# AndrewCullacino/handwritten-chinese-ocr-samples

Hardware: AMD Instinct MI355X
Metric: text-lines/sec (1x128x2000 synth) greedy decode (higher is better)
Workload: dtype f16 (f32 accumulate); 1 GPU; BASELINE configs[1]: 64 x 1x128x2000 uint8 lines, random-init hctr checkpoint (C=7358), forward + greedy CTC decode, labels to host; global_lines=64, lines_per_gpu=64, width=2000, classes=7358, checkpoint=random, parallelism=batch-shard x1

## Files before the change

### handwritten-chinese-ocr-samples_amd/_lib.py

```python
import ctypes
import os
import subprocess
import sys

PKG_DIR = os.path.dirname(os.path.abspath(__file__))
ROOT = os.path.dirname(PKG_DIR)
CSRC = os.path.join(PKG_DIR, "csrc")
LIB_PATH = os.path.join(PKG_DIR, "libhctr_hip.so")
HEADER = os.path.join(ROOT, "include", "hctr_hip.h")

SOURCES = [("gather.cpp", ["-x", "hip"]), ("kernels.hip", []), ("preprocess.hip", ["-ffp-contract=off"]), ("engine.cpp", ["-x", "hip"]), ("beam_search.cpp", ["-ffp-contract=off"]),
           ("ngram_lm.cpp", ["-ffp-contract=off"])]
COMMON = ["--offload-arch=gfx950", "-O3", "-std=c++17", "-fPIC", "-Wall", "-Wno-unused-function"]

HCTR_OK = 0
ERR_ARG, ERR_HIP, ERR_STATE, ERR_KEY, ERR_SHAPE, ERR_EMPTY_LINE, ERR_NOMEM = -1, -2, -3, -4, -5, -6, -7
U8, F32, I64 = 0, 1, 2


def _deps():
    return [os.path.join(CSRC, s) for s, _ in SOURCES] + [os.path.join(CSRC, "kernels.h"),
                                                          os.path.join(CSRC, "ngram_lm.h"), HEADER]


# ... 92 lines not shown
LM_NEXT_CB = ctypes.CFUNCTYPE(ctypes.c_int, ctypes.c_void_p, ctypes.c_int, c_i32p, c_i32p, ctypes.c_int, c_i32p)


class BeamParams(ctypes.Structure):
    _fields_ = [("skip_search", ctypes.c_int), ("beam_size", ctypes.c_int), ("search_depth", ctypes.c_int),
                ("lm_panelty", ctypes.c_double), ("len_bonus", ctypes.c_double),
                ("builtin_lm", ctypes.c_int), ("label_codepoints", ctypes.c_void_p),
                ("score_cb", LM_SCORE_CB), ("next_cb", LM_NEXT_CB), ("user", ctypes.c_void_p),
                ("num_threads", ctypes.c_int), ("ngram", ctypes.c_void_p), ("label_words", ctypes.c_void_p)]


_VP, _I, _I64 = ctypes.c_void_p, ctypes.c_int, ctypes.c_int64
SIGNATURES = [
    ("hctr_create", _I, [ctypes.POINTER(_VP), _I, _I]),
    ("hctr_destroy", None, [_VP]),
    ("hctr_last_error", ctypes.c_char_p, [_VP]),
    ("hctr_version", ctypes.c_char_p, []),
    ("hctr_load_tensor", _I, [_VP, ctypes.c_char_p, _VP, c_i64p, _I, _I]),
    ("hctr_finalize_weights", _I, [_VP]),
    ("hctr_set_precision", _I, [_VP, _I]),
    ("hctr_set_guard", _I, [_VP, ctypes.c_double, ctypes.c_double]),
    ("hctr_last_guard", _I, [_VP, c_i64p, c_i64p, _VP, _VP, _VP, _I64]),
    ("hctr_lines_per_pass", _I, [_VP, _I, _I, _I]),
    ("hctr_workspace_stats", _I, [_VP, c_i64p, c_i64p, c_i64p]),
    ("hctr_forward_logits", _I, [_VP, _VP, _I, _I, _VP, _I, _I, _VP, _I]),
    ("hctr_greedy", _I, [_VP, _VP, _I, _I, _VP, _I, _I, _VP, _VP]),
    ("hctr_decode_greedy_logits", _I, [_VP, _VP, _I, _I, _I, _I, _VP, _VP]),
    ("hctr_beam_frontend", _I, [_VP, _VP, _I, _I, _VP, _VP, _I, _I, _I, _I, _I, _I, _VP, _VP, _VP, c_i64p]),
    ("hctr_beam_fetch_candidates", _I, [_VP, _VP, _VP, _VP]),
    ("hctr_log_softmax", _I, [_VP, _VP, _I, _I, _I, _I, _VP]),
    ("hctr_ctc_loss", _I, [_VP, _VP, _I, _I, _VP, _I, _I, _VP, _VP, _VP, _VP]),
    ("hctr_ctc_loss_logits", _I, [_VP, _VP, _I, _I, _I, _I, _VP, _VP, _VP, _VP]),
    ("hctr_ctc_loss_logits_grad", _I, [_VP, _VP, _I, _I, _I, _I, _VP, _VP, _VP, _VP, _VP, _VP, _I]),
    ("hctr_ctc_align", _I, [_VP, _VP, _I, _I, _VP, _I, _I, _VP, _VP, _VP, _VP, _VP, _VP, _VP, _VP]),
    ("hctr_ctc_align_logits", _I, [_VP, _VP, _I, _I, _I, _I, _VP, _VP, _VP, _VP, _VP, _VP, _VP, _VP]),
    ("hctr_recognize", _I, [_VP, _VP, _I, _I, _VP, _I, _I, _VP, _VP, _VP, _VP, _VP, _VP, _VP, _VP, _VP]),
    ("hctr_recognize_logits", _I, [_VP, _VP, _I, _I, _I, _I, _VP, _VP, _VP, _VP, _VP, _VP, _VP, _VP, _VP]),
    ("hctr_beam_search", _I, [ctypes.POINTER(BeamParams), _I, _I, _I, _I, _VP, _VP, _VP, _VP, _VP, _VP, _VP,
                              _VP, _VP, _VP]),
    ("hctr_ngram_load", _I, [ctypes.c_char_p, ctypes.POINTER(_VP)]),
    ("hctr_ngram_free", None, [_VP]),
    ("hctr_ngram_order", _I, [_VP]),
    ("hctr_ngram_word_id", ctypes.c_int32, [_VP, ctypes.c_char_p]),
    ("hctr_ngram_score", ctypes.c_double, [_VP, ctypes.c_char_p, _I, _I]),
    ("hctr_ngram_last_error", ctypes.c_char_p, []),
    ("hctr_comm_unique_id", _I, [_VP]),
# ... 83 lines not shown
```

### handwritten-chinese-ocr-samples_amd/csrc/engine.cpp

```cpp
#include "../../include/hctr_hip.h"
#include "kernels.h"

#include <algorithm>
#include <cfloat>
#include <cmath>
#include <cstdarg>
#include <cstdio>
#include <cstring>
#include <map>
#include <new>
#include <string>
#include <vector>

using namespace hctr;

namespace {

constexpr int kImgH = 128;
constexpr int kFeat = 2048;
constexpr double kBnEps = 1e-5;
constexpr int kStagePlanes[4] = {128, 256, 512, 512};
constexpr int kStageBlocks[4] = {2, 4, 5, 1};
constexpr int kStageH[5] = {128, 64, 32, 16, 8};
constexpr int64_t kDefaultMaxCols = 131072;
// ... 107 lines not shown
    bool big_tiles = true;
    int halo_mode = 2;
    int mode = 0;
    bool split = false;
    int x3_mask = 31;
    int out_class = 8;
    double guard_rel = 0.01, guard_abs = 0.05;
    std::vector<float> g_margin, g_scale;
    std::vector<uint8_t> g_flag;
    int64_t g_flagged_total = 0, g_lines_total = 0;
    std::vector<std::vector<int32_t>> h_widths;
    std::vector<int32_t> h_labels, h_lengths;
    char* pin = nullptr;
    size_t pin_cap = 0;
    int chm() const { return split ? 3 : 1; }
    bool fuse_se = true;
    std::string stamp_layer;
    unsigned long long* stamp_buf = nullptr;
    int64_t stamp_cap = 0, stamp_n = 0;
    bool fuse_ds = true;
    bool fuse_argmax = true;
    bool persist_dynamic = false;
    int conv_seq = 0;
    bool fuse_stem = true;
    bool fuse_beam = true;
    int64_t beam_fallbacks = 0;
    bool profiling = false;
    std::vector<ProfEntry> prof;
    std::vector<hipEvent_t> ev_pool;
    size_t ev_used = 0;
    std::vector<void*> beam_allocs;
    std::vector<int64_t> cand_off;
    std::vector<int32_t> cand_idx;
    std::vector<float> cand_logp;
    char* ctc_buf = nullptr;
    size_t ctc_cap = 0;
};

namespace {

int fail(hctr_ctx* c, int code, const char* fmt, ...) {
    char buf[1024];
    va_list ap;
    va_start(ap, fmt);
    vsnprintf(buf, sizeof(buf), fmt, ap);
    va_end(ap);
// ... 452 lines not shown
        a.ds_in_sh = ws.Wa * ds->cin;
        a.ds_in_sb = (int64_t)(in.H + 2) * ws.Wa * ds->cin;
    }
    a.mtiles = ws.B * a.tilesH * a.tilesW;
    a.ntiles = cw.coutPad / conv_tile_couts(tile);
    if (c->persist_dynamic && c->conv_seq < 64) a.tile_counter = ws.tile_ctrs + 8 * c->conv_seq++;
    if (c->stamp_buf && c->stamp_layer == name && (tile == TILE_HALO4 || tile == TILE_HALO4_8x32) &&
        (int64_t)a.mtiles * a.ntiles <= c->stamp_cap) {
        a.stamps = c->stamp_buf;
        c->stamp_n = (int64_t)a.mtiles * a.ntiles;
    }
    static const char* dbg_layer = getenv("HCTR_DBG_LAYER");
    if (dbg_layer && strcmp(dbg_layer, name) == 0)
        if (const char* e = getenv("HCTR_DBG")) a.dbg = atoi(e);
    pf.begin(name);
    if (stem_img_f32 >= 0) {
        if (tile != TILE_64x256 || cw.taps != 9 || cw.cin != 64 || cw.coutPad != 64 || c->split)
            return fail(c, HCTR_ERR_STATE, "conv %s: stem fusion not applicable", name);
        a.img = ws.img; a.img_f32 = stem_img_f32; a.img_widths = stem_widths ? ws.widths : nullptr;
        a.stem_w = c->wts().stem_w; a.stem_b = c->wts().stem_b;
        HIP_TRY(c, launch_stem_conv0_2(a, c->stream));
    } else {
        HIP_TRY(c, launch_conv(a, tile, cw.taps, false, c->stream));
    }
    pf.end();
    return HCTR_OK;
}

int run_block(hctr_ctx* c, Prof& pf, const std::string& name, const BlockW& bw, ActDesc in, half_t* t,
              half_t* o, half_t* r, int planes) {
    const Workspace& ws = c->ws;
    const int H = in.H;
    auto tiles_of = [&](const ConvW& cw) {
        const ConvTile t = pick_tile(c, cw, H);
        return (H / conv_tile_rows(t)) * ((ws.W + conv_tile_cols(t) - 1) / conv_tile_cols(t));
    };
    const float inv_hw = 1.0f / ((float)H * (float)ws.W);
    const half_t* res = in.p;
    const bool fuse_ds = bw.has_ds && c->fuse_ds && (c->fuse_se || c->split) && bw.ds.cin % kBK == 0 &&
                         pick_tile(c, bw.conv2, H) == TILE_HALO4;
    if (bw.has_ds && !fuse_ds) {
        c->out_class = 4;
        TRY(run_conv(c, pf, (name + ".downsample").c_str(), bw.ds, in, r, H, false, false, nullptr, false));
        res = r;
    }
    if (c->fuse_se || c->split) {
// ... 720 lines not shown

int hctr_last_guard(hctr_ctx* c, int64_t* lines, int64_t* flagged, uint8_t* flags, float* min_margin, float* scale,
                    int64_t cap) {
    return guard(c, [&]() -> int {
        if (!c) return HCTR_ERR_ARG;
        const int64_t n = (int64_t)c->g_flag.size();
        int64_t nf = 0;
        for (uint8_t f : c->g_flag) nf += f ? 1 : 0;
        if (lines) *lines = n;
        if (flagged) *flagged = nf;
        const int64_t m = n < cap ? n : (cap < 0 ? 0 : cap);
        if (flags && m) memcpy(flags, c->g_flag.data(), (size_t)m);
        if (min_margin && m) memcpy(min_margin, c->g_margin.data(), (size_t)m * 4);
        if (scale && m) memcpy(scale, c->g_scale.data(), (size_t)m * 4);
        return HCTR_OK;
    });
}

int hctr_workspace_stats(hctr_ctx* c, int64_t* arena_bytes, int64_t* arena_allocations, int64_t* recarves) {
    if (!c) return HCTR_ERR_ARG;
    if (arena_bytes) *arena_bytes = (int64_t)c->arena_cap;
    if (arena_allocations) *arena_allocations = c->arena_reallocs;
    if (recarves) *recarves = c->ws_recarves;
    return HCTR_OK;
}

int hctr_lines_per_pass(hctr_ctx* c, int B, int W, int f16x3) {
    return guard(c, [&]() -> int {
        if (!c) return HCTR_ERR_ARG;
        if (B < 1 || W < 1) return fail(c, HCTR_ERR_ARG, "bad batch shape B=%d W=%d", B, W);
        return sub_batch(c, B, W, f16x3 != 0);
    });
}

int hctr_set_profiling(hctr_ctx* c, int enabled) {
    if (!c) return HCTR_ERR_ARG;
    c->profiling = enabled != 0;
    return HCTR_OK;
}

int hctr_last_profile(hctr_ctx* c, char* names_buf, int cap, float* ms, int max_n) {
    return guard(c, [&]() -> int {
        if (!c) return HCTR_ERR_ARG;
        HIP_TRY(c, hipStreamSynchronize(c->stream));
        std::string names;
        std::vector<std::string> order;
// ... 809 lines not shown
```

### handwritten-chinese-ocr-samples_amd/csrc/kernels.h

```cpp
#pragma once
#include <hip/hip_runtime.h>
#include <stdint.h>

namespace hctr {

typedef _Float16 half_t;

constexpr int kTileW = 16;
constexpr int kBK = 64;

struct ConvArgs {
    const half_t* x;
    const half_t* w;
    const float* bias;
    void* y;
    float* se_part;
    const float* se_scale;
    const half_t* resid;
    int H, W;
    int Cin, Cout, CoutPad;
    int tilesW, tilesH;
    int64_t in_sb;
    int in_sh;
    int64_t out_sb;
// ... 23 lines not shown
    const float* stem_w;
    const float* stem_b;
    int split;
    int drop_lo;
    const half_t* ds_x;
    const half_t* ds_w;
    const float* ds_bias;
    int ds_cin;
    int ds_in_sh;
    int64_t ds_in_sb;
    int32_t* tile_counter;
    unsigned long long* stamps;
    int dbg;
};

enum ConvTile { TILE_64x256 = 0, TILE_128x128 = 1, TILE_256x256 = 2, TILE_HALO4 = 3, TILE_HALO4_8x32 = 4 };
inline int conv_tile_rows(ConvTile t) { return (t == TILE_128x128 || t == TILE_HALO4_8x32) ? 8 : 16; }
inline int conv_tile_cols(ConvTile t) { return t == TILE_HALO4_8x32 ? 32 : 16; }
inline int conv_tile_couts(ConvTile t) {
    return t == TILE_64x256 ? 64 : (t == TILE_256x256 ? 256 : 128);
}

hipError_t launch_conv(const ConvArgs& a, ConvTile tile, int taps, bool linear_f32, hipStream_t s);
constexpr int kLinearWN = 2;
hipError_t launch_argmax_partials(const float* val, const int32_t* cls, int P, int64_t M, int32_t* idx, hipStream_t s,
                                  const float* val2 = nullptr, const float* absp = nullptr, float* margin = nullptr,
                                  float* rowabs = nullptr);
hipError_t launch_row_guard(const float* logits, int64_t ld, int64_t M, int C, float* margin, float* rowabs, hipStream_t s);
hipError_t launch_line_guard(const float* margin, const float* rowabs, int B, int W, float* out, hipStream_t s);
size_t conv_lds_bytes(ConvTile tile);

hipError_t launch_stem_conv0_2(const ConvArgs& a, hipStream_t s);

hipError_t launch_zero_borders(half_t* p, int B, int H, int W, int Wa, int C, hipStream_t s);

hipError_t launch_stem(const void* img, int img_f32, const int32_t* widths_dev, const float* w9,
                       const float* bias, half_t* y, int B, int W, int Wa, int split, hipStream_t s);

hipError_t launch_se_border(const half_t* t, int B, int H, int W, int Wa, int C, int split, const float* tsum_part,
                            int tiles, float* out, hipStream_t s);
hipError_t launch_se_premean(const float* border, const half_t* t, const half_t* w, const float* bias, int B, int H,
                             int W, int Wa, int C, int CoutPad, int split, float* mean, const float* w1,
                             const float* w2, float* scale, int32_t* counter, hipStream_t s);

hipError_t launch_se_fc(const float* se_part, int tiles_per_img, const float* w1, const float* w2,
                        float* scale, int B, int C, float inv_hw, hipStream_t s);
// ... 86 lines not shown
```

### handwritten-chinese-ocr-samples_amd/csrc/kernels.hip

```cpp
#include "kernels.h"

#include <algorithm>
#include <cstdlib>

namespace hctr {

typedef _Float16 f16x8 __attribute__((ext_vector_type(8)));
typedef float f32x4 __attribute__((ext_vector_type(4)));
typedef float f32x2 __attribute__((ext_vector_type(2)));
typedef _Float16 f16x2 __attribute__((ext_vector_type(2)));
typedef uint32_t u32x4 __attribute__((ext_vector_type(4)));
typedef void __attribute__((address_space(3))) * lptr_t;

__device__ __forceinline__ void glds16_asm(const char* gsrc, char* lds_dst) {
    const uint32_t lds = (uint32_t)(uintptr_t)((lptr_t)lds_dst);
    uint32_t keep;
    asm volatile("s_mov_b32 %0, m0\n\ts_mov_b32 m0, %2\n\ts_nop 0\n\tglobal_load_lds_dwordx4 %1, off\n\ts_mov_b32 m0, %0"
                 : "=&s"(keep)
                 : "v"(gsrc), "s"(lds)
                 : "memory");
}

template <int CTRL>
__device__ __forceinline__ float dpp_f32(float v) {
// ... 27 lines not shown
                 : "v"(voff), "s"(s0), "s"(s1), "s"(s2), "s"(s3), "s"(l0), "s"(l1), "s"(l2), "s"(l3)
                 : "memory");
}

template <int LSTRIDE>
__device__ __forceinline__ void glds16x4v_asm_s(const char* sbase, uint32_t v0, uint32_t v1, uint32_t v2, uint32_t v3, char* d0) {
    const uint32_t l0 = (uint32_t)(uintptr_t)((lptr_t)d0);
    uint32_t keep;
    asm volatile("s_mov_b32 %0, m0\n\t"
                 "s_mov_b32 m0, %6\n\ts_nop 0\n\tglobal_load_lds_dwordx4 %1, %5\n\t"
                 "s_add_u32 m0, m0, %7\n\ts_nop 0\n\tglobal_load_lds_dwordx4 %2, %5\n\t"
                 "s_add_u32 m0, m0, %7\n\ts_nop 0\n\tglobal_load_lds_dwordx4 %3, %5\n\t"
                 "s_add_u32 m0, m0, %7\n\ts_nop 0\n\tglobal_load_lds_dwordx4 %4, %5\n\t"
                 "s_mov_b32 m0, %0"
                 : "=&s"(keep)
                 : "v"(v0), "v"(v1), "v"(v2), "v"(v3), "s"(sbase), "s"(l0), "i"(LSTRIDE)
                 : "memory", "scc");
}

__device__ __forceinline__ constexpr int acc_cout_offset(int j) { return (j >> 2) * 64 + ((j >> 1) & 1) * 32 + (j & 1) * 4; }

constexpr float kSeScaleFloor = 1e-12f;

template <int WN, int WM, int JT, bool LINEAR, bool SPLIT, bool PRIVATE_RED = false, bool BIAS_DONE = false,
          bool RESID_IN_ACC = false>
__device__ __forceinline__ void conv_epilogue(const ConvArgs& a, f32x4 (&acc)[JT][4], char* smem, int tid, int lane,
                                              int wn, int wm, int n0, int mt, int img, int th, int tw, int hbase,
                                              int w0, unsigned long long* st = nullptr) {
    auto estamp = [&](int i) {
        if (st != nullptr) {
            __builtin_amdgcn_sched_barrier(0);
            if (tid == 0) st[i] = __builtin_amdgcn_s_memrealtime();
            __builtin_amdgcn_sched_barrier(0);
        }
    };
    constexpr int WC = JT * 16;
    constexpr int BN = WN * WC, BM = WM * 64;
    const int q = lane >> 4;
    const int c = lane & 15;
    const int cw0 = n0 + wn * WC + q * 8;
    auto co = [](int j) { return acc_cout_offset(j); };

    if (!BIAS_DONE) {
#pragma unroll
        for (int j = 0; j < JT; ++j) {
            const f32x4 b4 = *(const f32x4*)(a.bias + cw0 + co(j));
#pragma unroll
            for (int n = 0; n < 4; ++n)
#pragma unroll
                for (int i = 0; i < 4; ++i) acc[j][n][i] += b4[i];
        }
// ... 130 lines not shown
            for (int cb = 0; cb < JT / 4; ++cb)
#pragma unroll
                for (int n = 0; n < 4; ++n) {
                    const half_t* r = a.resid + pix0 + (int64_t)(hbase + n) * a.out_sh + cb * 64;
                    const f16x8 h0 = *(const f16x8*)r, h1 = *(const f16x8*)(r + 32);
                    const f16x8 l0 = *(const f16x8*)(r + a.Cout), l1 = *(const f16x8*)(r + a.Cout + 32);
#pragma unroll
                    for (int e = 0; e < 16; ++e) {
                        const float rv = e < 8 ? (float)h0[e] + (float)l0[e] : (float)h1[e - 8] + (float)l1[e - 8];
                        const float sv = sc[cb * 64 + (e >> 3) * 32 + (e & 7)];
                        acc[cb * 4 + (e >> 2)][n][e & 3] = fmaf(acc[cb * 4 + (e >> 2)][n][e & 3], sv, rv);
                    }
                }
        }
    } else if (RESID_IN_ACC) {
        const float* sc = a.se_scale + (int64_t)img * a.Cout + cw0;
#pragma unroll
        for (int j = 0; j < JT; ++j) {
            const f32x4 s4 = *(const f32x4*)(sc + co(j));
#pragma unroll
            for (int n = 0; n < 4; ++n)
#pragma unroll
                for (int i = 0; i < 4; ++i) acc[j][n][i] *= fmaxf(s4[i], kSeScaleFloor);
        }
    } else if (a.se_scale != nullptr) {
        const float* sc = a.se_scale + (int64_t)img * a.Cout + cw0;
        if (w < a.out_wlimit) {
            f16x8 rlo[JT / 4][4], rhi[JT / 4][4];
#pragma unroll
            for (int cb = 0; cb < JT / 4; ++cb)
#pragma unroll
                for (int n = 0; n < 4; ++n) {
                    const half_t* r = a.resid + pix0 + (int64_t)(hbase + n) * a.out_sh + cb * 64;
                    rlo[cb][n] = *(const f16x8*)r;
                    rhi[cb][n] = *(const f16x8*)(r + 32);
                }
#pragma unroll
            for (int j = 0; j < JT; ++j) {
                const f32x4 s4 = *(const f32x4*)(sc + co(j));
#pragma unroll
                for (int n = 0; n < 4; ++n)
#pragma unroll
                    for (int i = 0; i < 4; ++i) {
                        const int e = (j & 3) * 4 + i;
                        const float r = e < 8 ? (float)rlo[j >> 2][n][e] : (float)rhi[j >> 2][n][e - 8];
                        acc[j][n][i] = fmaf(acc[j][n][i], s4[i], r);
// ... 562 lines not shown
                __builtin_amdgcn_s_setprio(0);
                __builtin_amdgcn_sched_barrier(0);
            }
        }
    }
    asm volatile("s_waitcnt vmcnt(0)" ::: "memory");
    conv_epilogue<WN, WM, JT, false, false>(a, acc, smem, tid, lane, wn, wm, n0, mt, img, th, tw, th * 16 + wm * 4,
                                            tw * 16);
}

namespace halo4_lds {
constexpr int kWeightBuf = 16384;
constexpr int kWeights = 0;
constexpr int kHalo = kWeights + 2 * kWeightBuf;
constexpr int kScratch = kHalo + kHaloBytes;
constexpr int kScratchBytes = 4 * 128 * 4;
constexpr int kHaloTable = kScratch;
constexpr int kHaloTableBytes = 4 * 12 * 8 * 4;
constexpr int kNextTile = kScratch + kScratchBytes;
constexpr int kTotal = kNextTile + 16;
static_assert(kHaloTableBytes <= kScratchBytes, "the halo-offset table fits inside the epilogue scratch it aliases");
static_assert(kNextTile >= kScratch + kScratchBytes, "the next-tile words lie behind the epilogue scratch");
static_assert(kTotal <= 80 * 1024, "two workgroups per CU on 160 KB of LDS");
}

template <int GEOM, bool SPLIT, bool PERSIST, bool STAMP = false, bool DSFUSE = false, bool RESPRE = false>
__global__ __launch_bounds__(256, 2) void conv3x3_halo4_kernel(const ConvArgs a) {
    static_assert(!DSFUSE || !PERSIST, "downsample fusion: non-persistent instances only");
    static_assert(!RESPRE || (!DSFUSE && !PERSIST && !SPLIT), "residual-in-prologue: plain f16 instances only");
    constexpr int WN = 1, WM = 4, JT = 8, BN = 128;
    constexpr int TR = GEOM ? 8 : 16, TC = GEOM ? 32 : 16;
    constexpr int S = TC + 4;
    static_assert((TR + 2) * S * 128 == kHaloBytes, "halo footprint");
    extern __shared__ __attribute__((aligned(16))) char smem[];
    const int tid = threadIdx.x;
    auto stamp = [&](int i) {
        if (STAMP && tid == 0) a.stamps[(size_t)blockIdx.x * 16 + i] = __builtin_amdgcn_s_memrealtime();
    };
    stamp(0);
    const int lane = tid & 63;
    const int wv = __builtin_amdgcn_readfirstlane(tid >> 6);
    const int wm = wv;
    const int cin = a.Cin;
    const int nkc = (a.dbg & 64) ? 0 : cin / kBK;
    const int nk = 9 * nkc;
    constexpr bool kPrefetch = !PERSIST && !STAMP && !RESPRE;
    static_assert(!(kPrefetch && PERSIST), "the halo-offset table aliases the epilogue scratch: one tile per workgroup");
    constexpr int kRing = 3;
    constexpr int kBhalfAt = 1;
    constexpr int kBpreAt = 4;
    constexpr int kEarlyAt = 1;

// ... 84 lines not shown
#pragma unroll
            for (int r = 0; r < 12; ++r) htab[(wv * 12 + r) * 8 + (lane >> 3)] = hoff[r] - cp0;
        }
    };
    const int hbuf = halo4_lds::kHalo + wrow * (S * 128);
    int bx[3][2];
#pragma unroll
    for (int d = 0; d < 3; ++d) {
        const int u = wcol + c + d;
        const int v0 = u * 128 + (((q ^ (u & 7)) & 7) << 4);
        bx[d][0] = hbuf + v0;
        bx[d][1] = hbuf + (v0 ^ 64);
    }
    auto b_ptrs = [&](int tap, const char*& be, const char*& bo) {
        const int tdy = tap / 3, d = tap - tdy * 3;
        be = smem + bx[d][tdy & 1] + tdy * (S * 128);
        bo = smem + bx[d][(tdy & 1) ^ 1] + tdy * (S * 128);
    };

    Tile cur = tile_at(tidx);
    int kbase = 0;
    bool first = true;

    int tile_no = 0;
    for (;;) {
        const bool has_next = PERSIST && (tnext < xcnt);
        const char* nxb = cur.xb;
        const char* nwb = cur.wb;
        if (has_next) {
            const Tile t = tile_at(tnext);
            nxb = t.xb;
            nwb = t.wb;
        }
        int drawn = 0;
        if (dynamic && tid == 0)
            drawn = 2 * nloc + __hip_atomic_fetch_add(a.tile_counter + xcd, 1, __ATOMIC_RELAXED, __HIP_MEMORY_SCOPE_AGENT);
        f32x4 acc[JT][4];
        f16x8 bq[2][4];
        auto mma_step = [&](const char* wt, const char* be, const char* bo, auto&& stage_next, auto&& after_group,
                            bool have_b0 = false, const char* nbe = nullptr, const char* nbo = nullptr,
                            int bhalf_at = kBhalfAt) {
            f16x8 ar[kRing][2];
            auto read_a = [&](int g, f16x8 (&dst)[2]) {
                const int ks = g >> 2, jp = g & 3;
                const char* base = wt + (ks ? aoff1 : aoff0);
                dst[0] = *(const f16x8*)(base + (2 * jp) * 2048);
// ... 143 lines not shown

        __builtin_amdgcn_s_waitcnt(0xc07f);
        __builtin_amdgcn_s_setprio(1);
        for (int kc = 0; kc < nkc; ++kc) {
            const bool next_chunk = kc + 1 < nkc;
#pragma unroll
            for (int tap = 0; tap < 9; ++tap) {
                const int k = kc * 9 + tap;
                asm volatile("s_waitcnt vmcnt(0)" ::: "memory");
                if (!(a.dbg & 1024)) __builtin_amdgcn_s_barrier();
                asm volatile("" ::: "memory");
                const char *be, *bo;
                b_ptrs(tap, be, bo);
                const bool more = k + 1 < nk;
                const bool wrap = tap == 8;
                const int tap1 = more ? (wrap ? 0 : tap + 1) : 0;
                const int kc1 = more ? (wrap ? kc + 1 : kc) : 0;
                const char* wsrc = more ? cur.wb : nwb;
                const char *nbe = nullptr, *nbo = nullptr;
                if (kPrefetch && tap < 8) b_ptrs(tap + 1, nbe, nbo);
                mma_step(weight_buf(kbase + k), be, bo, [&] {
                    if ((more || has_next) && !(a.dbg & 512))
                        stage_weights(wsrc, kc1, tap1, (kbase + k + 1) & 1);
                }, [&](int g) {
                    if (kPrefetch && tap == 8 && g == kEarlyAt && next_chunk) {
                        asm volatile("s_waitcnt lgkmcnt(0)" ::: "memory");
                        __builtin_amdgcn_s_barrier();
                        asm volatile("" ::: "memory");
                        static_assert(kHaloPieces == 45, "halo piece count");
                        const char* hsrc = (next_chunk ? cur.xb + (int64_t)(kc + 1) * (kBK * 2) : nxb);
                        char* d = smem + halo4_lds::kHalo + wv * 1024;
                        int ln = lane;
                        asm volatile("" : "+v"(ln));
                        const uint32_t* hrow = (const uint32_t*)(smem + halo4_lds::kHaloTable) + wv * 96 + (ln >> 3);
                        const uint32_t cpl = (uint32_t)((ln ^ (ln >> 3)) & 7) << 4;
                        uint32_t ho[4];
#pragma unroll
                        for (int r = 0; r < 4; ++r) ho[r] = hrow[r * 8] + cpl;
                        glds16x4v_asm_s<4096>(hsrc, ho[0], ho[1], ho[2], ho[3], d);
#pragma unroll
                        for (int r = 0; r < 4; ++r) ho[r] = hrow[(4 + r) * 8] + cpl;
                        glds16x4v_asm_s<4096>(hsrc, ho[0], ho[1], ho[2], ho[3], d + 4 * 4096);
#pragma unroll
                        for (int r = 0; r < 4; ++r) ho[r] = hrow[(8 + r) * 8] + cpl;
#pragma unroll
                        for (int r = 8; r < 11; ++r) glds16_asm_s(hsrc, ho[r - 8], d + r * 4096);
                        if (wv == 0) glds16_asm_s(hsrc, ho[3], d + 11 * 4096);
                    }
                }, kPrefetch && tap > 0, nbe, nbo, (kPrefetch && tap == 8) ? 0 : kBhalfAt);
            }
            if (!kPrefetch && (next_chunk || has_next) && !(a.dbg & 32)) {
                __builtin_amdgcn_s_barrier();
                asm volatile("" ::: "memory");
                if (next_chunk) stage_halo(cur.xb, kc + 1);
                else stage_halo(nxb, 0);
            }
        }
        __builtin_amdgcn_s_setprio(0);
        stamp(3);
        if (a.dbg & 128) {
            float t = 0.f;
#pragma unroll
            for (int j = 0; j < JT; ++j)
#pragma unroll
                for (int n = 0; n < 4; ++n) t += acc[j][n][0] + acc[j][n][1] + acc[j][n][2] + acc[j][n][3];
            if (t == 123.456f) ((half_t*)a.y)[0] = (half_t)t;
        } else
        {
            const int tw = cur.tw, th = cur.th, img = cur.img;
            conv_epilogue<WN, WM, JT, false, SPLIT, true, true, DSFUSE || RESPRE>(
                a, acc, smem + halo4_lds::kScratch, tid, lane, 0, wm, cur.n0, cur.mt, img, th, tw, th * TR + wrow,
                tw * TC + wcol, STAMP ? a.stamps + (size_t)blockIdx.x * 16 : nullptr);
        }
        if (!has_next) break;
        kbase += nk;
        tidx = tnext;
        if (dynamic) {
            if (tid == 0) lds_next[tile_no & 1] = drawn;
            __builtin_amdgcn_s_waitcnt(0xc07f);
            __builtin_amdgcn_s_barrier();
            tnext = __builtin_amdgcn_readfirstlane(lds_next[tile_no & 1]);
        } else {
            tnext = tidx + nloc;
        }
        ++tile_no;
        cur = tile_at(tidx);
    }
    if (a.dbg & 64) asm volatile("s_waitcnt vmcnt(0)" ::: "memory");
    if (STAMP) {
        stamp(4);
        asm volatile("s_waitcnt vmcnt(0)" ::: "memory");
        stamp(5);
        if (tid == 0) {
            a.stamps[(size_t)blockIdx.x * 16 + 6] = __builtin_amdgcn_s_getreg((31 << 11) | 4);
            a.stamps[(size_t)blockIdx.x * 16 + 7] = __builtin_amdgcn_s_getreg((31 << 11) | 20);
// ... 151 lines not shown
            }
            halo_prev = halo_now;
            __builtin_amdgcn_sched_barrier(0);
#pragma unroll
            for (int g = 0; g < 8; ++g) {
                if (g + 2 < 8) read_a(g + 2, ar[(g + 2) % 3]);
                __builtin_amdgcn_sched_barrier(0);
                if (g == 1) { read_b(1, bq[1]); __builtin_amdgcn_sched_barrier(0); }
#pragma unroll
                for (int jj = 0; jj < 2; ++jj)
#pragma unroll
                    for (int n = 0; n < 4; ++n)
                        acc[2 * (g & 3) + jj][n] = __builtin_amdgcn_mfma_f32_16x16x32_f16(ar[g % 3][jj], bq[g >> 2][n],
                                                                                         acc[2 * (g & 3) + jj][n], 0, 0, 0);
                __builtin_amdgcn_sched_barrier(0);
            }
        }
    }
    __builtin_amdgcn_s_setprio(0);
    conv_epilogue<WN, WM, JT, false, false, true, true, false>(a, acc, smem + halo4_lds::kScratch, tid, lane, 0, wm, n0, mt, img, th, tw,
                                                               th * TR + wrow, tw * TC + wcol);
}

template <auto KERNEL>
static hipError_t launch_halo4_instance(const ConvArgs& a0, int grid, hipStream_t s, bool with_env_dbg = true) {
    static bool done[64] = {};
    hipError_t e0 = raise_lds_limit((const void*)KERNEL, halo4_lds::kTotal, done);
    if (e0 != hipSuccess) return e0;
    static const int dbg = env_dbg();
    ConvArgs a = a0;
    if (with_env_dbg) a.dbg |= dbg;
    hipLaunchKernelGGL(KERNEL, dim3(grid), dim3(256), halo4_lds::kTotal, s, a);
    return hipGetLastError();
}

template <int GEOM, bool SPLIT, bool PERSIST>
static hipError_t launch_conv_halo4_tp(const ConvArgs& a, hipStream_t s) {
    int grid = a.mtiles * a.ntiles;
    if (PERSIST) {
        static int cus[64] = {};
        int dev = 0;
        (void)hipGetDevice(&dev);
        if (dev >= 0 && dev < 64 && cus[dev] == 0) {
            hipDeviceProp_t prop;
            if (hipGetDeviceProperties(&prop, dev) == hipSuccess) cus[dev] = prop.multiProcessorCount;
            if (cus[dev] <= 0) cus[dev] = 256;
        }
        const int resident = 2 * ((dev >= 0 && dev < 64) ? cus[dev] : 256);
        if (grid > resident) grid = resident;
        grid = (grid + 7) / 8 * 8;
    }
    return launch_halo4_instance<conv3x3_halo4_kernel<GEOM, SPLIT, PERSIST>>(a, grid, s);
}
template <int GEOM, bool SPLIT>
static hipError_t launch_conv_halo4_t(const ConvArgs& a, hipStream_t s) {
    const int grid = a.mtiles * a.ntiles;
    if (a.ds_x != nullptr) {
        if (GEOM != 0) return hipErrorInvalidValue;
        return launch_halo4_instance<conv3x3_halo4_kernel<0, SPLIT, false, false, true>>(a, grid, s);
    }
    if (a.stamps != nullptr && !SPLIT)
        return launch_halo4_instance<conv3x3_halo4_kernel<GEOM, false, false, true>>(a, grid, s, false);
    static const int persist = [] { const char* e = getenv("HCTR_PERSIST"); return e ? atoi(e) : 0; }();
    if constexpr (!SPLIT) {
        static const int respre = [] { const char* e = getenv("HCTR_RESPRE"); return e ? atoi(e) : 0; }();
        if (respre && persist == 0 && a.resid != nullptr && a.se_scale != nullptr)
            return launch_halo4_instance<conv3x3_halo4_kernel<GEOM, false, false, false, false, true>>(a, grid, s);
    }
    if (persist == 0 || (persist == 2 && a.tile_counter == nullptr)) return launch_conv_halo4_tp<GEOM, SPLIT, false>(a, s);
    ConvArgs b = a;
    if (persist != 2) b.tile_counter = nullptr;
    return launch_conv_halo4_tp<GEOM, SPLIT, true>(b, s);
}
template <int GEOM>
static hipError_t launch_conv_halo4(const ConvArgs& a0, hipStream_t s) {
    ConvArgs a = a0;
    auto shift_of = [](int v) { int sft = 0; while ((1 << sft) < v) ++sft; return (1 << sft) == v ? sft : -1; };
    a.nt_shift = shift_of(a.ntiles);
    a.th_shift = shift_of(a.tilesH);
    if (a.tilesW < 1 || (uint64_t)a.mtiles * (uint64_t)a.tilesW >= ((uint64_t)1 << 40)) return hipErrorInvalidValue;
    a.tw_magic = (((uint64_t)1 << 40) + (uint64_t)a.tilesW - 1) / (uint64_t)a.tilesW;
    static const bool halfhalo = [] { const char* e = getenv("HCTR_HALFHALO"); return e ? atoi(e) != 0 : false; }();
    static const int persist = [] { const char* e = getenv("HCTR_PERSIST"); return e ? atoi(e) : 0; }();
    if (halfhalo && !a.split && a.ds_x == nullptr && a.stamps == nullptr && persist == 0 && a.Cin % kBK == 0)
        return launch_halo4_instance<conv3x3_halo4h_kernel<GEOM>>(a, a.mtiles * a.ntiles, s);
    return a.split ? launch_conv_halo4_t<GEOM, true>(a, s) : launch_conv_halo4_t<GEOM, false>(a, s);
}

static hipError_t launch_conv_halo(const ConvArgs& a, hipStream_t s) {
    static bool done[64] = {};
// ... 1885 lines not shown
```

### handwritten-chinese-ocr-samples_amd/model.py

```python
import collections
import ctypes

import numpy as np

from . import _lib

IncompatibleKeys = collections.namedtuple("IncompatibleKeys", ["missing_keys", "unexpected_keys"])
_PRECISIONS = {"f16": 0, "f16x3": 1, "auto": 2}


def _is_torch(x):
    return hasattr(x, "data_ptr") and hasattr(x, "is_cuda")


class hctr_model(object):
    def __init__(self, num_classes=7375, precision="f16"):
        if precision not in _PRECISIONS:
            raise ValueError("precision must be 'f16', 'f16x3' or 'auto'")
        self.precision = precision
        self.img_height = 128
        self.PAD = 'NormalizePAD'
        self.optimizer = 'SGD'
        self.pred = 'CTC'
        self.noutput = num_classes
# ... 240 lines not shown
        if n < 0:
            _lib.check(n, self._ctx)
        return n

    def workspace_stats(self):
        a, n, r = ctypes.c_int64(0), ctypes.c_int64(0), ctypes.c_int64(0)
        _lib.check(_lib.load().hctr_workspace_stats(self._require_ctx(), ctypes.byref(a), ctypes.byref(n), ctypes.byref(r)),
                   self._ctx)
        return {"arena_bytes": int(a.value), "arena_allocations": int(n.value), "recarves": int(r.value)}

    def set_profiling(self, enabled=True):
        _lib.check(_lib.load().hctr_set_profiling(self._require_ctx(), int(enabled)), self._ctx)

    def last_profile(self):
        ctx = self._require_ctx()
        names = ctypes.create_string_buffer(1 << 14)
        ms = (ctypes.c_float * 256)()
        n = _lib.load().hctr_last_profile(ctx, names, len(names), ms, 256)
        if n < 0:
            _lib.check(n, ctx)
        nm = names.value.decode().split("\n")
        return [(nm[i], float(ms[i])) for i in range(n)]

    def debug_activation(self, name, batch):
        ctx = self._require_ctx()
        lib = _lib.load()
        C, H = ctypes.c_int(), ctypes.c_int()
        n = lib.hctr_debug_activation(ctx, name.encode(), None, 0, ctypes.byref(C), ctypes.byref(H))
        if n < 0:
            _lib.check(int(n), ctx)
        out = np.empty((n,), dtype=np.float32)
        n2 = lib.hctr_debug_activation(ctx, name.encode(), _lib.ptr(out), n, ctypes.byref(C), ctypes.byref(H))
        if n2 < 0:
            _lib.check(int(n2), ctx)
        return out.reshape(batch, C.value, H.value, -1)


def beam_frontend_call(ctx, x, dt, on_dev, widths, logits, logits_on_dev, B, W, C, k, want_candidates):
    lib = _lib.load()
    topk_idx = np.empty((W, B, k), dtype=np.int32)
    topk_logp = np.empty((W, B, k), dtype=np.float32)
    blank = np.empty((W, B), dtype=np.float32)
    ncand = ctypes.c_int64(0)
    _lib.check(lib.hctr_beam_frontend(ctx, _lib.ptr(x), dt, on_dev, _lib.ptr(widths), _lib.ptr(logits), logits_on_dev,
                                      B, W, C, k, int(bool(want_candidates)), _lib.ptr(topk_idx), _lib.ptr(topk_logp),
                                      _lib.ptr(blank), ctypes.byref(ncand)), ctx)
# ... 11 lines not shown
```

### include/hctr_hip.h

```cpp
#ifndef HCTR_HIP_H
#define HCTR_HIP_H

#include <stdint.h>

#ifdef __cplusplus
extern "C" {
#endif

typedef struct hctr_ctx hctr_ctx;

typedef enum {
    HCTR_OK = 0,
    HCTR_ERR_ARG = -1,
    HCTR_ERR_HIP = -2,
    HCTR_ERR_STATE = -3,
    HCTR_ERR_KEY = -4,
    HCTR_ERR_SHAPE = -5,
    HCTR_ERR_EMPTY_LINE = -6,
    HCTR_ERR_NOMEM = -7
} hctr_status;

typedef enum { HCTR_U8 = 0, HCTR_F32 = 1, HCTR_I64 = 2 } hctr_dtype;

int hctr_create(hctr_ctx** out, int device, int num_classes);
// ... 87 lines not shown
int hctr_beam_search(const hctr_beam_params* p, int W, int B, int C, int k,
                     const int32_t* topk_idx, const float* topk_logp, const float* blank_logp,
                     const int64_t* cand_off, const int32_t* cand_idx, const float* cand_logp,
                     const float* full_logp_wbc,
                     int32_t* out_labels, int32_t* out_lengths, int32_t* line_status);

int hctr_resize_lines(hctr_ctx* ctx, const uint8_t* packed_src, int64_t packed_bytes, const int64_t* offsets,
                      const int32_t* heights, const int32_t* widths, const int32_t* channels, int n,
                      int out_height, const int32_t* out_widths, int out_W, uint8_t* out, int out_on_device);

#define HCTR_COMM_ID_BYTES 128
typedef struct hctr_comm hctr_comm;
int hctr_comm_unique_id(void* id128);
int hctr_comm_create(hctr_comm** out, const void* id128, int rank, int world, int device);
void hctr_comm_destroy(hctr_comm* comm);
int hctr_gather_labels(hctr_comm* comm, const int32_t* labels, const int32_t* lengths, int n_local, int row_stride,
                       int lines_per_rank, int cap, int32_t* out_labels, int32_t* out_lengths);
const char* hctr_comm_last_error(void);

int hctr_set_profiling(hctr_ctx* ctx, int enabled);
int hctr_last_profile(hctr_ctx* ctx, char* names_buf, int cap, float* ms, int max_n);
int hctr_workspace_stats(hctr_ctx* ctx, int64_t* arena_bytes, int64_t* arena_allocations, int64_t* recarves);
int hctr_lines_per_pass(hctr_ctx* ctx, int B, int W, int f16x3);
int64_t hctr_debug_stamps(hctr_ctx* ctx, const char* layer, uint64_t* out, int64_t cap_wgs);

int64_t hctr_debug_activation(hctr_ctx* ctx, const char* name, float* out, int64_t cap,
                              int* C, int* H);

#ifdef __cplusplus
}
#endif
#endif
```

Baseline: 518.4 lines/s.

## Stage residual tile into LDS via async DMA during final conv taps

Adds a RESLDS variant of the halo4 3x3 conv kernel that prefetches the residual tile into LDS with global-to-LDS loads. Row 0 goes into the idle weight buffer and rows 1..3 go into the halo region, both during the last tap. The epilogue then reads the residual from LDS with a swizzled layout and fuses the SE-scale and residual add, which removes the dependent global residual loads from the epilogue. It is on by default for eligible non-split layers, with an env switch, and the LDS request grows to 80 KB. Debug counters and a map export are added for testing.

New measurement: 519.8 lines/s (median of 6 runs). Within noise of the previous version (+0.3%).

```diff
diff --git a/handwritten-chinese-ocr-samples_amd/_lib.py b/handwritten-chinese-ocr-samples_amd/_lib.py
--- a/handwritten-chinese-ocr-samples_amd/_lib.py
+++ b/handwritten-chinese-ocr-samples_amd/_lib.py
@@ -138,6 +138,8 @@
     ("hctr_set_guard", _I, [_VP, ctypes.c_double, ctypes.c_double]),
     ("hctr_last_guard", _I, [_VP, c_i64p, c_i64p, _VP, _VP, _VP, _I64]),
     ("hctr_lines_per_pass", _I, [_VP, _I, _I, _I]),
+    ("hctr_resid_lds_launches", _I64, [_VP]),
+    ("hctr_resid_lds_map", _I, [_I, _I, _I, _I, _I, _I, c_i32p]),
     ("hctr_workspace_stats", _I, [_VP, c_i64p, c_i64p, c_i64p]),
     ("hctr_forward_logits", _I, [_VP, _VP, _I, _I, _VP, _I, _I, _VP, _I]),
     ("hctr_greedy", _I, [_VP, _VP, _I, _I, _VP, _I, _I, _VP, _VP]),
diff --git a/handwritten-chinese-ocr-samples_amd/csrc/engine.cpp b/handwritten-chinese-ocr-samples_amd/csrc/engine.cpp
--- a/handwritten-chinese-ocr-samples_amd/csrc/engine.cpp
+++ b/handwritten-chinese-ocr-samples_amd/csrc/engine.cpp
@@ -153,6 +153,7 @@
     bool fuse_argmax = true;
     bool persist_dynamic = false;
     int conv_seq = 0;
+    int64_t resid_lds_launches = 0;
     bool fuse_stem = true;
     bool fuse_beam = true;
     int64_t beam_fallbacks = 0;
@@ -651,6 +652,7 @@
         HIP_TRY(c, launch_stem_conv0_2(a, c->stream));
     } else {
         HIP_TRY(c, launch_conv(a, tile, cw.taps, false, c->stream));
+        if (cw.taps == 9 && conv_takes_resid_lds(a, tile)) ++c->resid_lds_launches;
     }
     pf.end();
     return HCTR_OK;
@@ -1417,6 +1419,16 @@
     if (arena_bytes) *arena_bytes = (int64_t)c->arena_cap;
     if (arena_allocations) *arena_allocations = c->arena_reallocs;
     if (recarves) *recarves = c->ws_recarves;
+    return HCTR_OK;
+}
+
+int64_t hctr_resid_lds_launches(hctr_ctx* c) { return c ? c->resid_lds_launches : HCTR_ERR_ARG; }
+
+int hctr_resid_lds_map(int geom, int wave, int out_sh, int out_sw, int cols_valid, int idle_buf, int32_t* out) {
+    if (geom < 0 || geom > 1 || wave < 0 || wave > 3 || out_sh < 1 || out_sw < 128 || out_sw % 128 != 0 || idle_buf < 0 ||
+        idle_buf > 1 || !out)
+        return HCTR_ERR_ARG;
+    resid_lds_map(geom, wave, out_sh, out_sw, cols_valid, idle_buf, out);
     return HCTR_OK;
 }
 
diff --git a/handwritten-chinese-ocr-samples_amd/csrc/kernels.h b/handwritten-chinese-ocr-samples_amd/csrc/kernels.h
--- a/handwritten-chinese-ocr-samples_amd/csrc/kernels.h
+++ b/handwritten-chinese-ocr-samples_amd/csrc/kernels.h
@@ -69,6 +69,8 @@
 }
 
 hipError_t launch_conv(const ConvArgs& a, ConvTile tile, int taps, bool linear_f32, hipStream_t s);
+bool conv_takes_resid_lds(const ConvArgs& a, ConvTile tile);
+void resid_lds_map(int geom, int wave, int out_sh, int out_sw, int cols_valid, int idle, int32_t* out);
 constexpr int kLinearWN = 2;
 hipError_t launch_argmax_partials(const float* val, const int32_t* cls, int P, int64_t M, int32_t* idx, hipStream_t s,
                                   const float* val2 = nullptr, const float* absp = nullptr, float* margin = nullptr,
diff --git a/handwritten-chinese-ocr-samples_amd/csrc/kernels.hip b/handwritten-chinese-ocr-samples_amd/csrc/kernels.hip
--- a/handwritten-chinese-ocr-samples_amd/csrc/kernels.hip
+++ b/handwritten-chinese-ocr-samples_amd/csrc/kernels.hip
@@ -73,11 +73,18 @@
 
 constexpr float kSeScaleFloor = 1e-12f;
 
+namespace halo4_lds {
+constexpr int kResidPixel = 256;
+constexpr int kResidRow = 16 * kResidPixel;
+__host__ __device__ constexpr int resid_read_off(int c, int k) { return c * kResidPixel + (((k ^ c) & 15) << 4); }
+}
+
 template <int WN, int WM, int JT, bool LINEAR, bool SPLIT, bool PRIVATE_RED = false, bool BIAS_DONE = false,
-          bool RESID_IN_ACC = false>
+          bool RESID_IN_ACC = false, bool RESID_LDS = false>
 __device__ __forceinline__ void conv_epilogue(const ConvArgs& a, f32x4 (&acc)[JT][4], char* smem, int tid, int lane,
                                               int wn, int wm, int n0, int mt, int img, int th, int tw, int hbase,
-                                              int w0, unsigned long long* st = nullptr) {
+                                              int w0, unsigned long long* st = nullptr, const char* rl0 = nullptr,
+                                              const char* rl1 = nullptr) {
     auto estamp = [&](int i) {
         if (st != nullptr) {
             __builtin_amdgcn_sched_barrier(0);
@@ -254,6 +261,37 @@
             for (int n = 0; n < 4; ++n)
 #pragma unroll
                 for (int i = 0; i < 4; ++i) acc[j][n][i] *= fmaxf(s4[i], kSeScaleFloor);
+        }
+    } else if (RESID_LDS) {
+        const float* sc = a.se_scale + (int64_t)img * a.Cout + cw0;
+        f32x4 s4[JT];
+#pragma unroll
+        for (int j = 0; j < JT; ++j) s4[j] = *(const f32x4*)(sc + co(j));
+        asm volatile("s_waitcnt vmcnt(0)" ::: "memory");
+        if (w < a.out_wlimit) {
+            int ln = lane;
+            asm volatile("" : "+v"(ln));
+            const int rq = ln >> 4, rc = ln & 15;
+            f16x8 rlo[JT / 4][4], rhi[JT / 4][4];
+#pragma unroll
+            for (int cb = 0; cb < JT / 4; ++cb)
+#pragma unroll
+                for (int n = 0; n < 4; ++n) {
+                    const char* r = n == 0 ? rl0 : rl1 + (n - 1) * halo4_lds::kResidRow;
+                    rlo[cb][n] = *(const f16x8*)(r + halo4_lds::resid_read_off(rc, cb * 8 + rq));
+                    rhi[cb][n] = *(const f16x8*)(r + halo4_lds::resid_read_off(rc, cb * 8 + 4 + rq));
+                }
+#pragma unroll
+            for (int j = 0; j < JT; ++j) {
+#pragma unroll
+                for (int n = 0; n < 4; ++n)
+#pragma unroll
+                    for (int i = 0; i < 4; ++i) {
+                        const int e = (j & 3) * 4 + i;
+                        const float r = e < 8 ? (float)rlo[j >> 2][n][e] : (float)rhi[j >> 2][n][e - 8];
+                        acc[j][n][i] = fmaf(acc[j][n][i], s4[j][i], r);
+                    }
+            }
         }
     } else if (a.se_scale != nullptr) {
         const float* sc = a.se_scale + (int64_t)img * a.Cout + cw0;
@@ -862,12 +900,64 @@
 static_assert(kHaloTableBytes <= kScratchBytes, "the halo-offset table fits inside the epilogue scratch it aliases");
 static_assert(kNextTile >= kScratch + kScratchBytes, "the next-tile words lie behind the epilogue scratch");
 static_assert(kTotal <= 80 * 1024, "two workgroups per CU on 160 KB of LDS");
-}
-
-template <int GEOM, bool SPLIT, bool PERSIST, bool STAMP = false, bool DSFUSE = false, bool RESPRE = false>
+
+constexpr int kResidRow0 = kWeights;
+constexpr int kResidRest = kHalo;
+constexpr int kResidEnd = kResidRest + 4 * 3 * kResidRow;
+constexpr int kTotalResid = 80 * 1024;
+static_assert(4 * kResidRow == kWeightBuf, "patch rows 0 of the four waves fill exactly the idle weight buffer");
+static_assert(kResidRest >= kWeights + 2 * kWeightBuf, "rows 1..3 lie behind both weight buffers (one is being read)");
+static_assert(kResidEnd <= kTotalResid && kTotalResid <= 80 * 1024, "the residual image ends inside 80 KB");
+static_assert(kTotalResid >= kTotal, "a RESLDS launch still holds the ordinary layout");
+
+__host__ __device__ constexpr int resid_row_lds(int wave, int n, int idle) {
+    return n == 0 ? kResidRow0 + idle * kWeightBuf + wave * kResidRow
+                  : kResidRest + (wave * 3 + (n - 1)) * kResidRow;
+}
+__host__ __device__ constexpr int resid_piece_lds(int wave, int p, int idle) { return resid_row_lds(wave, p >> 2, idle) + (p & 3) * 1024; }
+__host__ __device__ constexpr uint32_t resid_lane_voff(int lane, uint32_t sw_bytes) {
+    return (uint32_t)(lane >> 4) * sw_bytes + (uint32_t)(((lane & 15) ^ (lane >> 4)) << 4);
+}
+__host__ __device__ constexpr int resid_piece_col(int g, int cols_valid) {
+    const int last = cols_valid > 0 ? cols_valid - 1 : 0;
+    return 4 * g < last ? 4 * g : last;
+}
+__host__ __device__ constexpr int resid_piece_jmax(int g, int cols_valid) {
+    const int r = cols_valid - 1 - 4 * g;
+    return r < 0 ? 0 : (r > 3 ? 3 : r);
+}
+__host__ __device__ constexpr uint32_t resid_piece_voff(uint32_t voff0, int g, uint32_t jmax_bytes) {
+    const uint32_t v = voff0 ^ ((uint32_t)g << 6), lim = jmax_bytes | 0xF0u;
+    return v < lim ? v : lim;
+}
+}
+
+void resid_lds_map(int geom, int wave, int out_sh, int out_sw, int cols_valid, int idle, int32_t* out) {
+    const int wrow = geom ? (wave >> 1) * 4 : wave * 4, wcol = geom ? (wave & 1) * 16 : 0;
+    const uint32_t swb = (uint32_t)out_sw * 2u;
+    const int cv = cols_valid - wcol;
+    for (int p = 0; p < 16; ++p)
+        for (int l = 0; l < 64; ++l) {
+            const int n = p >> 2, g = p & 3;
+            const uint32_t v = halo4_lds::resid_piece_voff(halo4_lds::resid_lane_voff(l, swb), g,
+                                                           (uint32_t)halo4_lds::resid_piece_jmax(g, cv) * swb);
+            const int64_t goff = (int64_t)(wrow + n) * out_sh * 2 +
+                                 (int64_t)(wcol + halo4_lds::resid_piece_col(g, cv)) * swb + v;
+            int32_t* o = out + (p * 64 + l) * 4;
+            o[0] = n * 16 + 4 * g + (l >> 4);
+            o[1] = (int32_t)((v >> 4) & 15);
+            o[2] = halo4_lds::resid_piece_lds(wave, p, idle) + l * 16;
+            o[3] = (int32_t)goff;
+        }
+}
+
+template <int GEOM, bool SPLIT, bool PERSIST, bool STAMP = false, bool DSFUSE = false, bool RESPRE = false,
+          bool RESLDS = false>
 __global__ __launch_bounds__(256, 2) void conv3x3_halo4_kernel(const ConvArgs a) {
     static_assert(!DSFUSE || !PERSIST, "downsample fusion: non-persistent instances only");
     static_assert(!RESPRE || (!DSFUSE && !PERSIST && !SPLIT), "residual-in-prologue: plain f16 instances only");
+    static_assert(!RESLDS || (!DSFUSE && !PERSIST && !SPLIT && !STAMP && !RESPRE),
+                  "residual by LDS-DMA: plain f16 prefetching instances only");
     constexpr int WN = 1, WM = 4, JT = 8, BN = 128;
     constexpr int TR = GEOM ? 8 : 16, TC = GEOM ? 32 : 16;
     constexpr int S = TC + 4;
@@ -998,6 +1088,29 @@
     int kbase = 0;
     bool first = true;
 
+    const uint32_t rswb = RESLDS ? (uint32_t)a.out_sw * 2u : 0u;
+    const int rcv = RESLDS ? a.out_wlimit - (cur.tw * TC + wcol) : 0;
+    const int rsh = RESLDS ? a.out_sh : 0;
+    const char* rbase = RESLDS ? (const char*)(a.resid + a.out_off + cur.img * a.out_sb + (int64_t)(cur.tw * TC + wcol) * a.out_sw +
+                                               cur.n0 + (int64_t)(cur.th * TR + wrow) * a.out_sh)
+                               : nullptr;
+    auto stage_resid = [&](int nfrom, int nto, int idle) {
+        int ln = lane;
+        asm volatile("" : "+v"(ln));
+        const uint32_t v0 = halo4_lds::resid_lane_voff(ln, rswb);
+        int cv = rcv;
+        asm volatile("" : "+s"(cv));
+        uint32_t v[4];
+#pragma unroll
+        for (int g = 0; g < 4; ++g)
+            v[g] = halo4_lds::resid_piece_voff(v0, g, (uint32_t)halo4_lds::resid_piece_jmax(g, cv) * rswb) +
+                   (uint32_t)halo4_lds::resid_piece_col(g, cv) * rswb;
+#pragma unroll
+        for (int n = nfrom; n < nto; ++n)
+            glds16x4v_asm_s<1024>(rbase + (int64_t)n * rsh * 2, v[0], v[1], v[2], v[3],
+                                  smem + halo4_lds::resid_row_lds(wv, n, idle));
+    };
+
     int tile_no = 0;
     for (;;) {
         const bool has_next = PERSIST && (tnext < xcnt);
@@ -1187,11 +1300,16 @@
                 mma_step(weight_buf(kbase + k), be, bo, [&] {
                     if ((more || has_next) && !(a.dbg & 512))
                         stage_weights(wsrc, kc1, tap1, (kbase + k + 1) & 1);
+                    if (RESLDS && tap == 8 && !more) stage_resid(0, 1, (kbase + k + 1) & 1);
                 }, [&](int g) {
-                    if (kPrefetch && tap == 8 && g == kEarlyAt && next_chunk) {
+                    if (kPrefetch && tap == 8 && g == kEarlyAt && (next_chunk || RESLDS)) {
                         asm volatile("s_waitcnt lgkmcnt(0)" ::: "memory");
                         __builtin_amdgcn_s_barrier();
                         asm volatile("" ::: "memory");
+                        if (RESLDS && !next_chunk) {
+                            stage_resid(1, 4, 0);
+                            return;
+                        }
                         static_assert(kHaloPieces == 45, "halo piece count");
                         const char* hsrc = (next_chunk ? cur.xb + (int64_t)(kc + 1) * (kBK * 2) : nxb);
                         char* d = smem + halo4_lds::kHalo + wv * 1024;
@@ -1233,9 +1351,10 @@
         } else
         {
             const int tw = cur.tw, th = cur.th, img = cur.img;
-            conv_epilogue<WN, WM, JT, false, SPLIT, true, true, DSFUSE || RESPRE>(
+            conv_epilogue<WN, WM, JT, false, SPLIT, true, true, DSFUSE || RESPRE, RESLDS>(
                 a, acc, smem + halo4_lds::kScratch, tid, lane, 0, wm, cur.n0, cur.mt, img, th, tw, th * TR + wrow,
-                tw * TC + wcol, STAMP ? a.stamps + (size_t)blockIdx.x * 16 : nullptr);
+                tw * TC + wcol, STAMP ? a.stamps + (size_t)blockIdx.x * 16 : nullptr,
+                smem + halo4_lds::resid_row_lds(wv, 0, (kbase + nk) & 1), smem + halo4_lds::resid_row_lds(wv, 1, 0));
         }
         if (!has_next) break;
         kbase += nk;
@@ -1433,15 +1552,15 @@
                                                                th * TR + wrow, tw * TC + wcol);
 }
 
-template <auto KERNEL>
+template <auto KERNEL, int LDS = halo4_lds::kTotal>
 static hipError_t launch_halo4_instance(const ConvArgs& a0, int grid, hipStream_t s, bool with_env_dbg = true) {
     static bool done[64] = {};
-    hipError_t e0 = raise_lds_limit((const void*)KERNEL, halo4_lds::kTotal, done);
+    hipError_t e0 = raise_lds_limit((const void*)KERNEL, LDS, done);
     if (e0 != hipSuccess) return e0;
     static const int dbg = env_dbg();
     ConvArgs a = a0;
     if (with_env_dbg) a.dbg |= dbg;
-    hipLaunchKernelGGL(KERNEL, dim3(grid), dim3(256), halo4_lds::kTotal, s, a);
+    hipLaunchKernelGGL(KERNEL, dim3(grid), dim3(256), LDS, s, a);
     return hipGetLastError();
 }
 
@@ -1463,6 +1582,20 @@
     }
     return launch_halo4_instance<conv3x3_halo4_kernel<GEOM, SPLIT, PERSIST>>(a, grid, s);
 }
+bool conv_takes_resid_lds(const ConvArgs& a, ConvTile tile) {
+    static const int on = [] { const char* e = getenv("HCTR_RESLDS"); return e ? atoi(e) : 1; }();
+    static const int other = [] {
+        int n = 0;
+        for (const char* k : {"HCTR_PERSIST", "HCTR_RESPRE", "HCTR_HALFHALO"}) { const char* e = getenv(k); n |= e ? atoi(e) : 0; }
+        return n | env_dbg();
+    }();
+    if (!on || other || (tile != TILE_HALO4 && tile != TILE_HALO4_8x32)) return false;
+    if (a.out_wlimit <= (a.tilesW - 1) * conv_tile_cols(tile) + (tile == TILE_HALO4_8x32 ? 16 : 0)) return false;
+    return a.resid != nullptr && a.se_scale != nullptr && a.se_part == nullptr && !a.split && a.ds_x == nullptr &&
+           a.stamps == nullptr && a.dbg == 0 && !a.pool && a.Cin % kBK == 0 && a.Cin >= kBK && a.out_sw % 128 == 0 &&
+           a.CoutPad % 128 == 0;
+}
+
 template <int GEOM, bool SPLIT>
 static hipError_t launch_conv_halo4_t(const ConvArgs& a, hipStream_t s) {
     const int grid = a.mtiles * a.ntiles;
@@ -1477,6 +1610,11 @@
         static const int respre = [] { const char* e = getenv("HCTR_RESPRE"); return e ? atoi(e) : 0; }();
         if (respre && persist == 0 && a.resid != nullptr && a.se_scale != nullptr)
             return launch_halo4_instance<conv3x3_halo4_kernel<GEOM, false, false, false, false, true>>(a, grid, s);
+    }
+    if constexpr (!SPLIT) {
+        if (conv_takes_resid_lds(a, GEOM ? TILE_HALO4_8x32 : TILE_HALO4))
+            return launch_halo4_instance<conv3x3_halo4_kernel<GEOM, false, false, false, false, false, true>,
+                                         halo4_lds::kTotalResid>(a, grid, s);
     }
     if (persist == 0 || (persist == 2 && a.tile_counter == nullptr)) return launch_conv_halo4_tp<GEOM, SPLIT, false>(a, s);
     ConvArgs b = a;
diff --git a/handwritten-chinese-ocr-samples_amd/model.py b/handwritten-chinese-ocr-samples_amd/model.py
--- a/handwritten-chinese-ocr-samples_amd/model.py
+++ b/handwritten-chinese-ocr-samples_amd/model.py
@@ -286,6 +286,12 @@
         nm = names.value.decode().split("\n")
         return [(nm[i], float(ms[i])) for i in range(n)]
 
+    def resid_lds_launches(self):
+        n = _lib.load().hctr_resid_lds_launches(self._require_ctx())
+        if n < 0:
+            _lib.check(int(n), self._ctx)
+        return int(n)
+
     def debug_activation(self, name, batch):
         ctx = self._require_ctx()
         lib = _lib.load()
diff --git a/include/hctr_hip.h b/include/hctr_hip.h
--- a/include/hctr_hip.h
+++ b/include/hctr_hip.h
@@ -133,6 +133,8 @@
 int hctr_last_profile(hctr_ctx* ctx, char* names_buf, int cap, float* ms, int max_n);
 int hctr_workspace_stats(hctr_ctx* ctx, int64_t* arena_bytes, int64_t* arena_allocations, int64_t* recarves);
 int hctr_lines_per_pass(hctr_ctx* ctx, int B, int W, int f16x3);
+int64_t hctr_resid_lds_launches(hctr_ctx* ctx);
+int hctr_resid_lds_map(int geom, int wave, int out_sh, int out_sw, int cols_valid, int idle_buf, int32_t* out);
 int64_t hctr_debug_stamps(hctr_ctx* ctx, const char* layer, uint64_t* out, int64_t cap_wgs);
 
 int64_t hctr_debug_activation(hctr_ctx* ctx, const char* name, float* out, int64_t cap,
```
